# MinghanLi/STMask

Measured on AMD Instinct MI355X. Metric: frames/sec at 360x640 R50-DCN-FPN (STMask hot path, fp32), higher is better.
Workload: dtype f32

## Files before the change

stmask_amd/csrc/mask_ops.hip:

```cpp
#include "stm_common.h"

namespace {

constexpr int LC_DCHUNK = 32;

#ifndef LC_ABL
#define LC_ABL 0
#endif
template <int M>
__global__ __launch_bounds__(256) void lincomb_kernel(const float* __restrict__ proto, const float* __restrict__ coeff,
                                                      const float* __restrict__ boxes, float* __restrict__ out, int h,
                                                      int w, int n, int apply_tanh, const int* __restrict__ n_dev,
                                                      const int* __restrict__ row_proto, unsigned long long* __restrict__ bits,
                                                      float bits_thr, int dchunk)
{
    __shared__ float sc[LC_DCHUNK * M];
    __shared__ float sb[LC_DCHUNK * 4];
    const int hw = h * w;
    const int pix = blockIdx.x * 256 + threadIdx.x;
    const int d0 = blockIdx.y * dchunk;
    const int nd = min(dchunk, n - d0);
    const int n_valid = n_dev ? min(max(*n_dev, 0), n) : n;

    for (int idx = threadIdx.x; idx < nd * M; idx += 256) {
        float v = coeff[(int64_t)d0 * M + idx];
        sc[idx] = apply_tanh ? tanhf(v) : v;
    }
    if (threadIdx.x < nd) {
        float x1 = 0.f, x2 = (float)w, y1 = 0.f, y2 = (float)h;
        if (boxes) {
            const float* b = boxes + (int64_t)(d0 + threadIdx.x) * 4;
            stm_sanitize(b[0], b[2], w, 1, x1, x2);
            stm_sanitize(b[1], b[3], h, 1, y1, y2);
        }
        sb[threadIdx.x * 4 + 0] = x1;
        sb[threadIdx.x * 4 + 1] = x2;
        sb[threadIdx.x * 4 + 2] = y1;
        sb[threadIdx.x * 4 + 3] = y2;
    }
    __shared__ int hit[LC_DCHUNK];
    const int p0 = blockIdx.x * 256;
    const bool vec_ok = (hw & 3) == 0 && (reinterpret_cast<uintptr_t>(out) & 15) == 0;
    if (threadIdx.x < nd) {
        const int d = threadIdx.x;
        const int pl = min(p0 + 255, hw - 1);
        const int ya = p0 / w, yb = pl / w;
        const float fya = (float)ya, fyb = (float)yb;
        bool touch = (d0 + d < n_valid) && fyb >= sb[d * 4 + 2] && fya < sb[d * 4 + 3];
        if (touch && ya == yb) {
            const float fxa = (float)(p0 - ya * w), fxb = (float)(pl - ya * w);
            touch = fxb >= sb[d * 4] && fxa < sb[d * 4 + 1];
        }
        hit[d] = (touch || !vec_ok) ? 1 : 0;
    }
    __syncthreads();
    const bool live = pix < hw;
    const int words = (hw + 63) >> 6;
    if (p0 < hw) {
        const int lane = threadIdx.x & 63, wv = threadIdx.x >> 6;
        const int q = p0 + 4 * lane;
        for (int d = wv; d < nd; d += 4) {
            if (hit[d]) continue;
            if (q < hw && !(LC_ABL & 2)) *reinterpret_cast<float4*>(out + (int64_t)(d0 + d) * hw + q) = make_float4(0.f, 0.f, 0.f, 0.f);
            if (bits && lane < 4 && (p0 >> 6) + lane < words && !(LC_ABL & 4)) bits[(int64_t)(d0 + d) * words + (p0 >> 6) + lane] = 0ull;
        }
    }
    if (!bits && !live) return;
    if (bits && ((pix & ~63) >= hw)) return;

    float p[M];
    int cur = -1;
    const int y = pix / w, x = pix - y * w;
    const float fx = (float)x, fy = (float)y;
    for (int d = 0; d < nd; ++d) {
        if (!hit[d]) continue;
        const int want = row_proto ? row_proto[d0 + d] : 0;
        if (want != cur && live) {
            cur = want;
            const float4* pr = reinterpret_cast<const float4*>(proto + ((int64_t)cur * hw + pix) * M);
#pragma unroll
            for (int q = 0; q < M / 4; ++q) {
                float4 v = (LC_ABL & 1) ? make_float4(0.01f * q, 0.02f, 0.03f, 0.04f) : pr[q];
                p[4 * q] = v.x; p[4 * q + 1] = v.y; p[4 * q + 2] = v.z; p[4 * q + 3] = v.w;
            }
        }
        float v = 0.0f;
        const bool inside = live && (d0 + d < n_valid) && fx >= sb[d * 4] && fx < sb[d * 4 + 1] && fy >= sb[d * 4 + 2] &&
                            fy < sb[d * 4 + 3];
        if (inside) {
            float acc = 0.0f;
#pragma unroll
            for (int k = 0; k < M; ++k) acc = fmaf(p[k], sc[d * M + k], acc);
            v = 1.0f / (1.0f + expf(-acc));
        }
        if (live && (!(LC_ABL & 2) || v == 12345.678f)) out[(int64_t)(d0 + d) * hw + pix] = v;
        if (bits && !(LC_ABL & 4)) {
            const unsigned long long bal = __ballot(v > bits_thr);
            if ((threadIdx.x & 63) == 0) bits[(int64_t)(d0 + d) * words + (pix >> 6)] = bal;
        }
    }
}

__global__ __launch_bounds__(256) void mask_pack_kernel(const float* __restrict__ m, unsigned long long* __restrict__ bits,
                                                        int hw, int words, float thr)
{
    const int wave = threadIdx.x >> 6, lane = threadIdx.x & 63;
    const int word = blockIdx.x * 4 + wave;
    const int i = blockIdx.y;
    if (word >= words) return;
    const int pix = word * 64 + lane;
    bool b = false;
    if (pix < hw) b = m[(int64_t)i * hw + pix] > thr;
    unsigned long long bal = __ballot(b);
    if (lane == 0) bits[(int64_t)i * words + word] = bal;
}

__global__ __launch_bounds__(256) void mask_iou_pairs_small_kernel(const unsigned long long* __restrict__ b1,
                                                             const unsigned long long* __restrict__ b2, int n2, int words,
                                                             float* __restrict__ out, const int* __restrict__ g1,
                                                             const int* __restrict__ g2)
{
    extern __shared__ unsigned long long arow[];
    const int i = blockIdx.y;
    const int gi = g1 ? g1[i] : 0;
    if (g2) {
        const int j = blockIdx.x * 256 + threadIdx.x;
        const bool mine = j < n2 && g2[j] == gi;
        if (!__syncthreads_or(mine ? 1 : 0)) {
            if (j < n2) out[(int64_t)i * n2 + j] = 0.0f;
            return;
        }
    }
    for (int t = threadIdx.x; t < words; t += 256) arow[t] = b1[(int64_t)i * words + t];
    __syncthreads();
    const int j = blockIdx.x * 256 + threadIdx.x;
    if (j >= n2) return;
    if (g2 && g2[j] != gi) { out[(int64_t)i * n2 + j] = 0.0f; return; }
    int inter = 0, a1 = 0, a2 = 0;
    const unsigned long long* q = b2 + (int64_t)j * words;
    for (int t = 0; t < words; ++t) {
        unsigned long long a = arow[t], b = q[t];
        inter += __popcll(a & b);
        a1 += __popcll(a);
        a2 += __popcll(b);
    }
    float fi = (float)inter, uni = ((float)a1 + (float)a2) - fi;
    out[(int64_t)i * n2 + j] = (uni == 0.0f) ? 0.0f : fi / uni;
}

constexpr int MIOU_R = 8, MIOU_LIST = 2048, MIOU_BIG_ROWS = 3072;
constexpr int MIOU_DYN_LDS = 46 * 1024;
__global__ __launch_bounds__(256) void mask_iou_pairs_kernel(const unsigned long long* __restrict__ b1,
                                                             const unsigned long long* __restrict__ b2, int n1, int n2, int words,
                                                             float* __restrict__ out, const int* __restrict__ g1,
                                                             const int* __restrict__ g2, int R)
{
    extern __shared__ unsigned long long arow[];
    __shared__ int a1_s[MIOU_R], gi_s[MIOU_R];
    const int i0 = blockIdx.x * R, nr = min(R, n1 - i0);
    const int tid = threadIdx.x, lane = tid & 63, wave = tid >> 6;
    for (int r = wave; r < MIOU_R; r += 4) {
        unsigned pa = 0;
        for (int t = lane; t < words && r < nr; t += 64) {
            const unsigned long long a = b1[(int64_t)(i0 + r) * words + t];
            arow[r * words + t] = a;
            pa += (unsigned)__popcll(a);
        }
        pa = stm_row16_sum(pa);
        const int tot = stm_wave_sum_rows(pa);
        if (lane == 0) { a1_s[r] = tot; gi_s[r] = r < nr ? (g1 ? g1[i0 + r] : 0) : -0x7fffffff; }
    }
    __syncthreads();
    int gi[MIOU_R];
#pragma unroll
    for (int r = 0; r < MIOU_R; ++r) gi[r] = gi_s[r];
    const int q = lane >> 4, sl = lane & 15;
    __shared__ int list_j[MIOU_LIST], list_m[MIOU_LIST], chunk_n[4], list_n;
    if (tid == 0) list_n = 0;
// ... 23 lines not shown
        __syncthreads();
    }
    const int nlist = min(list_n, MIOU_LIST);
    for (int p0 = wave * 4; p0 < nlist; p0 += 16) {
        const int pi = min(p0 + q, nlist - 1);
        const int jq = list_j[pi];
        const unsigned mq = (unsigned)list_m[pi];
        const unsigned long long* col = b2 + (int64_t)jq * words;
        unsigned hi[MIOU_R], lo = 0;
#pragma unroll
        for (int r = 0; r < MIOU_R; ++r) hi[r] = 0;
        for (int t0 = sl; t0 < words; t0 += 16 * 16) {
            unsigned long long c[16];
#pragma unroll
            for (int u = 0; u < 16; ++u) c[u] = t0 + 16 * u < words ? col[t0 + 16 * u] : 0ull;
#pragma unroll
            for (int u = 0; u < 16; ++u) {
                const int t = t0 + 16 * u;
                if (t < words) {
                    lo += (unsigned)__popcll(c[u]);
#pragma unroll
                    for (int r = 0; r < MIOU_R; ++r)
                        if (r < nr) hi[r] += (unsigned)__popcll(arow[r * words + t] & c[u]);
                }
            }
        }
        lo = stm_row16_sum(lo);
#pragma unroll
        for (int r = 0; r < MIOU_R; ++r) hi[r] = stm_row16_sum(hi[r]);
        if (sl < MIOU_R && p0 + q < nlist) {
            unsigned h = 0;
#pragma unroll
            for (int r = 0; r < MIOU_R; ++r)
                if (sl == r) h = hi[r];
            if (sl < nr && ((mq >> sl) & 1u)) {
                const float fi = (float)h, uni = ((float)a1_s[sl] + (float)lo) - fi;
                out[(int64_t)(i0 + sl) * n2 + jq] = (uni == 0.0f) ? 0.0f : fi / uni;
            }
        }
    }
    if (list_n > MIOU_LIST) {
        for (int j = 0, seen = 0; j < n2; ++j) {
            const int gj = g2 ? g2[j] : 0;
            unsigned match = 0;
#pragma unroll
            for (int r = 0; r < MIOU_R; ++r) match |= (unsigned)(r < nr && gj == gi[r]) << r;
            if (!match) continue;
            if (seen++ < MIOU_LIST) continue;
            if (wave != 0) continue;
            const unsigned long long* col = b2 + (int64_t)j * words;
            for (int r = 0; r < nr; ++r) {
                if (!((match >> r) & 1u)) continue;
                unsigned h = 0, o = 0;
                for (int t = lane; t < words; t += 64) { const unsigned long long c = col[t]; o += (unsigned)__popcll(c); h += (unsigned)__popcll(arow[r * words + t] & c); }
                const int hs = stm_wave_sum_rows(stm_row16_sum(h)), os = stm_wave_sum_rows(stm_row16_sum(o));
                if (lane == 0) {
                    const float fi = (float)hs, uni = ((float)a1_s[r] + (float)os) - fi;
                    out[(int64_t)(i0 + r) * n2 + j] = (uni == 0.0f) ? 0.0f : fi / uni;
                }
            }
        }
    }
}

}

extern "C" int stm_lincomb_sigmoid_crop_bits_f32(const float* proto, const float* coeff, const float* boxes, float* out, int h, int w, int m,
                                                 int n, int apply_tanh, const int* n_dev, const int* row_proto, uint64_t* bits, float bits_thr,
                                                 stm_stream_t stream);
extern "C" int stm_lincomb_sigmoid_crop_f32(const float* proto, const float* coeff, const float* boxes, float* out, int h,
                                            int w, int m, int n, int apply_tanh, const int* n_dev, const int* row_proto,
                                            stm_stream_t stream)
{
    return stm_lincomb_sigmoid_crop_bits_f32(proto, coeff, boxes, out, h, w, m, n, apply_tanh, n_dev, row_proto, nullptr, 0.5f, stream);
}

extern "C" int stm_lincomb_sigmoid_crop_bits_f32(const float* proto, const float* coeff, const float* boxes, float* out, int h, int w, int m,
                                                 int n, int apply_tanh, const int* n_dev, const int* row_proto, uint64_t* bits_out, float bits_thr,
                                                 stm_stream_t stream)
{
    unsigned long long* bits = reinterpret_cast<unsigned long long*>(bits_out);
    STM_REQUIRE(n >= 0, STM_EINVAL, "stm_lincomb_sigmoid_crop_f32: n=%d", n);
    if (n == 0) return STM_OK;
    STM_REQUIRE(proto && coeff && out, STM_ENULL, "stm_lincomb_sigmoid_crop_f32: proto/coeff/out must be non-NULL");
    STM_REQUIRE(h > 0 && w > 0, STM_EINVAL, "stm_lincomb_sigmoid_crop_f32: bad mask size %dx%d", h, w);
    STM_REQUIRE((uintptr_t)proto % 16 == 0, STM_EINVAL, "stm_lincomb_sigmoid_crop_f32: proto must be 16-byte aligned");
    const int dchunk = (int64_t)stm_cdiv((int64_t)h * w, 256) * stm_cdiv(n, 32) >= 2048 ? 32 : 8;
    dim3 grid(stm_cdiv((int64_t)h * w, 256), stm_cdiv(n, dchunk));
    STM_REQUIRE(grid.y <= 65535, STM_EINVAL, "stm_lincomb_sigmoid_crop_f32: n=%d too large", n);
    if (m == 32) {
        hipLaunchKernelGGL(lincomb_kernel<32>, grid, dim3(256), 0, stm_hs(stream), proto, coeff, boxes, out, h, w, n,
                           apply_tanh, n_dev, row_proto, bits, bits_thr, dchunk);
    } else if (m == 8) {
        hipLaunchKernelGGL(lincomb_kernel<8>, grid, dim3(256), 0, stm_hs(stream), proto, coeff, boxes, out, h, w, n,
                           apply_tanh, n_dev, row_proto, bits, bits_thr, dchunk);
    } else if (m == 64) {
        hipLaunchKernelGGL(lincomb_kernel<64>, grid, dim3(256), 0, stm_hs(stream), proto, coeff, boxes, out, h, w, n,
                           apply_tanh, n_dev, row_proto, bits, bits_thr, dchunk);
    } else {
        STM_REQUIRE(false, STM_EUNSUPPORTED, "stm_lincomb_sigmoid_crop_f32: mask_dim %d not in {8,32,64}", m);
    }
    STM_CHECK_LAUNCH("lincomb_kernel");
    return STM_OK;
}

extern "C" size_t stm_mask_iou_workspace_bytes(int n1, int n2, int hw)
{
    size_t words = (size_t)((hw + 63) / 64);
    return ((size_t)n1 + (size_t)n2) * words * 8 + 64;
}

extern "C" int stm_mask_iou_grouped_f32(const float* m1, int n1, const float* m2, int n2, int hw, float thr, float* out, const int* group1,
                                        const int* group2, void* workspace, size_t workspace_bytes, stm_stream_t stream);
extern "C" int stm_mask_iou_f32(const float* m1, int n1, const float* m2, int n2, int hw, float thr, float* out,
                                void* workspace, size_t workspace_bytes, stm_stream_t stream)
{
    return stm_mask_iou_grouped_f32(m1, n1, m2, n2, hw, thr, out, nullptr, nullptr, workspace, workspace_bytes, stream);
}

extern "C" int stm_mask_iou_grouped_f32(const float* m1, int n1, const float* m2, int n2, int hw, float thr, float* out, const int* group1,
                                        const int* group2, void* workspace, size_t workspace_bytes, stm_stream_t stream)
{
    STM_REQUIRE((group1 == nullptr) == (group2 == nullptr), STM_EINVAL, "stm_mask_iou_grouped_f32: give both group arrays or neither");
    STM_REQUIRE(n1 >= 0 && n2 >= 0 && hw > 0, STM_EINVAL, "stm_mask_iou_f32: bad sizes");
    if (n1 == 0 || n2 == 0) return STM_OK;
    STM_REQUIRE(m1 && m2 && out, STM_ENULL, "stm_mask_iou_f32: m1/m2/out must be non-NULL");
    STM_REQUIRE(workspace && workspace_bytes >= stm_mask_iou_workspace_bytes(n1, n2, hw), STM_EWORKSPACE,
                "stm_mask_iou_f32: workspace too small");
    STM_REQUIRE(n1 <= 65535 && n2 <= 65535, STM_EINVAL, "stm_mask_iou_f32: too many masks");

    const int words = (hw + 63) / 64;
    unsigned long long* b1 = reinterpret_cast<unsigned long long*>(workspace);
    unsigned long long* b2 = b1 + (size_t)n1 * words;
    hipLaunchKernelGGL(mask_pack_kernel, dim3(stm_cdiv(words, 4), n1), dim3(256), 0, stm_hs(stream), m1, b1, hw, words, thr);
    hipLaunchKernelGGL(mask_pack_kernel, dim3(stm_cdiv(words, 4), n2), dim3(256), 0, stm_hs(stream), m2, b2, hw, words, thr);
    STM_CHECK_LAUNCH("mask_pack_kernel");
    const int rows_wg = std::min(MIOU_R, MIOU_DYN_LDS / (words * 8));
    STM_REQUIRE(rows_wg >= 1, STM_EUNSUPPORTED, "stm_mask_iou_f32: a mask row of %d words does not fit the 46 KB of LDS the kernel stages rows in", words);
    if (n1 < STM_ENV_INT("STM_MIOU_BIG_ROWS", MIOU_BIG_ROWS))
        hipLaunchKernelGGL(mask_iou_pairs_small_kernel, dim3(stm_cdiv(n2, 256), n1), dim3(256), (size_t)words * 8, stm_hs(stream), b1, b2, n2, words, out, group1, group2);
    else
        hipLaunchKernelGGL(mask_iou_pairs_kernel, dim3(stm_cdiv(n1, rows_wg)), dim3(256), (size_t)rows_wg * words * 8, stm_hs(stream), b1,
                           b2, n1, n2, words, out, group1, group2, rows_wg);
    STM_CHECK_LAUNCH("mask_iou_pairs_kernel");
    return STM_OK;
}

extern "C" int stm_mask_iou_bits_f32(const uint64_t* bits1, int n1, const uint64_t* bits2, int n2, int hw, float* out, const int* group1,
                                     const int* group2, stm_stream_t stream)
{
    STM_REQUIRE((group1 == nullptr) == (group2 == nullptr), STM_EINVAL, "stm_mask_iou_bits_f32: give both group arrays or neither");
    STM_REQUIRE(n1 >= 0 && n2 >= 0 && hw > 0, STM_EINVAL, "stm_mask_iou_bits_f32: bad sizes");
    if (n1 == 0 || n2 == 0) return STM_OK;
    STM_REQUIRE(bits1 && bits2 && out, STM_ENULL, "stm_mask_iou_bits_f32: bits1/bits2/out must be non-NULL");
    STM_REQUIRE(n1 <= 65535 && n2 <= 65535, STM_EINVAL, "stm_mask_iou_bits_f32: too many masks");

    const int words = (hw + 63) / 64;
    const int rows_wg = std::min(MIOU_R, MIOU_DYN_LDS / (words * 8));
    STM_REQUIRE(rows_wg >= 1, STM_EUNSUPPORTED, "stm_mask_iou_bits_f32: a mask row of %d words does not fit the 46 KB of LDS the kernel stages rows in", words);
    if (n1 < STM_ENV_INT("STM_MIOU_BIG_ROWS", MIOU_BIG_ROWS))
        hipLaunchKernelGGL(mask_iou_pairs_small_kernel, dim3(stm_cdiv(n2, 256), n1), dim3(256), (size_t)words * 8, stm_hs(stream),
                           reinterpret_cast<const unsigned long long*>(bits1), reinterpret_cast<const unsigned long long*>(bits2), n2, words, out, group1, group2);
    else
        hipLaunchKernelGGL(mask_iou_pairs_kernel, dim3(stm_cdiv(n1, rows_wg)), dim3(256), (size_t)rows_wg * words * 8, stm_hs(stream),
                           reinterpret_cast<const unsigned long long*>(bits1), reinterpret_cast<const unsigned long long*>(bits2), n1, n2, words, out, group1,
                           group2, rows_wg);
    STM_CHECK_LAUNCH("mask_iou_pairs_kernel");
// ... 150 lines not shown
```

stmask_amd/ops.py:

```python
import ctypes
import os

import torch

from . import _lib
from ._lib import DeformGeom, StmError, c_p, call


def _pair(v):
    return (v, v) if isinstance(v, int) else tuple(v)


def _dev(*ts):
    for t in ts:
        if t is not None and not t.is_cuda:
            raise StmError("stmask_amd ops need tensors on the MI355X (got a CPU tensor); there is no CPU fallback")


def _f32c(t):
    if t.dtype != torch.float32:
        raise StmError(f"expected float32, got {t.dtype}")
    return t if t.is_contiguous() else t.contiguous()


# ... 516 lines not shown
def encode(matched, priors):
    _dev(matched, priors)
    matched, priors = _f32c(matched), _f32c(priors)
    if matched.dim() != 2 or matched.shape[1] != 4 or priors.shape != matched.shape:
        raise StmError(f"encode: matched {tuple(matched.shape)} and priors {tuple(priors.shape)} must both be [n, 4]")
    out = torch.empty_like(matched)
    call("stm_encode_boxes_f32", _p(matched), _p(priors), _p(out), matched.shape[0], _stream())
    return out


_match_offsets = {}


def match_offsets(counts, device):
    if len(counts) == 1:
        key = (device.index, counts[0])
        t = _match_offsets.get(key)
        if t is None:
            t = _match_offsets[key] = torch.tensor([0, counts[0]], dtype=torch.int32, device=device)
        return t
    acc = [0]
    for c in counts:
        acc.append(acc[-1] + int(c))
    return torch.tensor(acc, dtype=torch.int32).pin_memory().to(device, non_blocking=True)


def match_priors(boxes, labels, ids, counts, priors, conf, pos_thresh, neg_thresh, out=None, offsets=None, want_status=False):
    _dev(boxes, labels, ids, priors, conf)
    counts = [int(c) for c in counts]
    B, G_total, G_max = len(counts), sum(counts), max(counts) if counts else 0
    conf = conf.detach()
    boxes, priors, conf = _f32c(boxes), _f32c(priors), _f32c(conf)
    if conf.dim() == 2:
        conf = conf[None]
    if conf.dim() != 3 or conf.shape[0] != B:
        raise StmError(f"match_priors: conf {tuple(conf.shape)} for {B} images (expected [B, P, C])")
    P, C = conf.shape[1], conf.shape[2]
    if tuple(boxes.shape) != (G_total, 4) or labels.shape[0] != G_total or ids.shape[0] != G_total:
        raise StmError(f"match_priors: boxes {tuple(boxes.shape)}, labels {tuple(labels.shape)}, ids {tuple(ids.shape)} for {G_total} boxes")
    if tuple(priors.shape) not in ((P, 4), (B, P, 4)):
        raise StmError(f"match_priors: priors {tuple(priors.shape)} for P={P}, B={B}")
    labels, ids = labels.to(torch.int64).contiguous(), ids.to(torch.int64).contiguous()
    dev = conf.device
    if offsets is None:
        offsets = match_offsets(counts, dev)
    if out is None:
        out = (torch.empty(B, P, 4, dtype=torch.float32, device=dev), torch.empty(B, P, 4, dtype=torch.float32, device=dev),
               torch.empty(B, P, dtype=torch.int64, device=dev), torch.empty(B, P, dtype=torch.int64, device=dev),
               torch.empty(B, P, dtype=torch.int64, device=dev))
    else:
        for t, dt, shp in zip(out, (torch.float32,) * 2 + (torch.int64,) * 3, ((B, P, 4),) * 2 + ((B, P),) * 3):
            if t.dtype != dt or t.numel() != B * P * (4 if len(shp) == 3 else 1) or not t.is_contiguous() or t.device != dev:
                raise StmError(f"match_priors: output {tuple(t.shape)} {t.dtype} must be contiguous {dt} with the elements of {shp}")
    status = torch.empty(B, dtype=torch.int32, device=dev) if want_status else None
    nbytes = _lib.lib().stm_match_workspace_bytes(B, P, G_total, G_max)
    ws = _workspace(nbytes, dev, "match")
    call("stm_match_priors_f32", _p(boxes), _p(labels), _p(ids), _p(offsets), B, G_total, G_max, _p(priors), 1 if priors.dim() == 3 else 0, P,
         _p(conf), C, float(pos_thresh), float(neg_thresh), _p(out[0]), _p(out[1]), _p(out[2]), _p(out[3]), _p(out[4]), _p(status), _p(ws), nbytes,
         _stream())
    return tuple(out) + ((status,) if want_status else ())


def jaccard(a, b):
    _dev(a, b)
    a, b = _f32c(a), _f32c(b)
    out = torch.empty(a.shape[0], b.shape[0], dtype=torch.float32, device=a.device)
    call("stm_jaccard_f32", _p(a), a.shape[0], _p(b), b.shape[0], _p(out), _stream())
    return out


def jaccard_backward(grad_out, a, b, need_a=True, need_b=True):
    _dev(grad_out, a, b)
    go, a, b = _f32c(grad_out), _f32c(a), _f32c(b)
    if tuple(go.shape) != (a.shape[0], b.shape[0]):
        raise StmError(f"jaccard_backward: grad_out {tuple(go.shape)} != {(a.shape[0], b.shape[0])}")
    ga = torch.empty_like(a) if need_a else None
    gb = torch.empty_like(b) if need_b else None
    if ga is None and gb is None:
        return None, None
    call("stm_jaccard_backward_f32", _p(go), _p(a), a.shape[0], _p(b), b.shape[0], _p(ga), _p(gb), _stream())
    return ga, gb


def lincomb_sigmoid_crop_bits(proto, coeff, boxes, row_proto, thr=0.5, apply_tanh=True):
    _dev(proto, coeff, boxes, row_proto)
    proto, coeff = _f32c(proto), _f32c(coeff)
    assert proto.dim() == 4 and row_proto.dtype == torch.int32 and row_proto.numel() == coeff.shape[0]
    h, w, m = proto.shape[1:]
    n = coeff.shape[0]
    out = torch.empty(n, h, w, dtype=torch.float32, device=proto.device)
    bits = torch.empty(n, (h * w + 63) // 64, dtype=torch.int64, device=proto.device)
    call("stm_lincomb_sigmoid_crop_bits_f32", _p(proto), _p(coeff), _p(_f32c(boxes)), _p(out), h, w, m, n, 1 if apply_tanh else 0, c_p(0),
         _p(row_proto), _p(bits), thr, _stream())
    return out, bits


def mask_iou_bits(bits1, bits2, hw, group1=None, group2=None):
    _dev(bits1, bits2, group1, group2)
    n1, n2 = bits1.shape[0], bits2.shape[0]
    if n1 == 0 or n2 == 0:
        return torch.zeros(n1, n2, dtype=torch.float32, device=bits1.device)
    out = torch.empty(n1, n2, dtype=torch.float32, device=bits1.device)
    if bits1.dtype != torch.int64 or bits2.dtype != torch.int64 or bits1.shape[1] != (hw + 63) // 64 or bits2.shape[1] != bits1.shape[1]:
        raise StmError("mask_iou_bits: bit tables must be int64 [n, ceil(hw / 64)]")
    call("stm_mask_iou_bits_f32", _p(bits1.contiguous()), n1, _p(bits2.contiguous()), n2, hw, _p(out),
         _p(group1.contiguous()) if group1 is not None else c_p(0), _p(group2.contiguous()) if group2 is not None else c_p(0), _stream())
    return out


def lincomb_sigmoid_crop(proto, coeff, boxes=None, apply_tanh=True, n_dev=None, row_proto=None):
    _dev(proto, coeff, boxes, row_proto)
    proto, coeff = _f32c(proto), _f32c(coeff)
    if row_proto is not None:
        assert proto.dim() == 4 and row_proto.dtype == torch.int32 and row_proto.numel() == coeff.shape[0]
        h, w, m = proto.shape[1:]
    else:
        h, w, m = proto.shape
    n = coeff.shape[0]
    bx = _f32c(boxes) if boxes is not None else None
    out = torch.empty(n, h, w, dtype=torch.float32, device=proto.device)
    call("stm_lincomb_sigmoid_crop_f32", _p(proto), _p(coeff), _p(bx), _p(out), h, w, m, n, 1 if apply_tanh else 0, _p(n_dev), _p(row_proto),
         _stream())
    return out


def lincomb_sigmoid_crop_backward(grad_out, proto, coeff, boxes=None, apply_tanh=True, need_proto=True, need_coeff=True):
    _dev(grad_out, proto, coeff, boxes)
    go, proto, coeff = _f32c(grad_out), _f32c(proto), _f32c(coeff)
    h, w, m = proto.shape
    n = coeff.shape[0]
    if tuple(go.shape) != (n, h, w) or coeff.shape[1] != m or (boxes is not None and tuple(boxes.shape) != (n, 4)):
        raise StmError(f"lincomb_sigmoid_crop_backward: grad_out {tuple(go.shape)}, proto {tuple(proto.shape)}, coeff {tuple(coeff.shape)} do not match")
    gp = torch.empty_like(proto) if need_proto else None
    gc = torch.empty_like(coeff) if need_coeff else None
    if gp is None and gc is None:
        return None, None
    bx = _f32c(boxes) if boxes is not None else None
    need = _lib.lib().stm_lincomb_backward_workspace_bytes(n, h, w, m)
    ws = _workspace(need, proto.device, "lcb")
    call("stm_lincomb_backward_f32", _p(go), _p(proto), _p(coeff), _p(bx), _p(gp), _p(gc), h, w, m, n, 1 if apply_tanh else 0, _p(ws), ws.numel(),
         _stream())
    return gp, gc


def _mask_bce_args(who, pred, target, idx, grad_loss=None):
    if pred.dtype != torch.float32 or pred.dim() != 3:
        raise StmError(f"{who}: pred must be float32 [n,h,w], got {pred.dtype} {tuple(pred.shape)}")
    if target.dtype not in (torch.uint8, torch.bool, torch.float32) or target.dim() != 3:
        raise StmError(f"{who}: target must be uint8, bool or float32 [G,H,W], got {target.dtype} {tuple(target.shape)}")
    n, h, w = pred.shape
    G, H, W = target.shape
    if h > H or w > W:
        raise StmError(f"{who}: pred {h}x{w} is larger than the target {H}x{W} (downsampling is not supported)")
    if idx is None:
        if G != n:
            raise StmError(f"{who}: without idx row i uses target i, but pred has {n} rows and target {G}")
    elif idx.dtype != torch.int64 or idx.dim() != 1 or idx.numel() != n:
        raise StmError(f"{who}: idx must be int64 [{n}], got {idx.dtype} {tuple(idx.shape)}")
    if grad_loss is not None and (grad_loss.dtype != torch.float32 or tuple(grad_loss.shape) != (n,)):
        raise StmError(f"{who}: grad_loss must be float32 [{n}], got {grad_loss.dtype} {tuple(grad_loss.shape)}")
    _dev(pred, target, idx, grad_loss)
    target = target if target.is_contiguous() else target.contiguous()
    if target.dtype == torch.bool:
        target = target.view(torch.uint8)
    return _f32c(pred), target, (idx if idx is None or idx.is_contiguous() else idx.contiguous()), target.dtype == torch.float32


def mask_bce_upsampled(pred, target, idx=None):
    pred, target, idx, is_f32 = _mask_bce_args("mask_bce_upsampled", pred, target, idx)
    n, h, w = pred.shape
    G, H, W = target.shape
    loss = torch.empty(n, dtype=torch.float32, device=pred.device)
    if n == 0:
        return loss
    need = _lib.lib().stm_mask_bce_workspace_bytes(n, H, W)
    ws = _workspace(need, pred.device, "mbce")
    call("stm_mask_bce_upsampled_f32", _p(pred), _p(target), 1 if is_f32 else 0, _p(idx), _p(loss), n, h, w, G, H, W, _p(ws), ws.numel(), _stream())
# ... 1260 lines not shown
```

stmask_amd/pipeline.py:

```python
import os
import sys
import time

import torch
import torch.nn.functional as F

from . import fuse, ops, track_host
from .dist import DET_COLS
from .layers import Track_TF, generate_candidate
from .trunk import TrunkRunner, concurrent_side_streams, trunk_stream_count

ROI_CHUNKS = (256, 128, 64)


class _StageTimer:

    def __init__(self):
        self.on = os.environ.get("STM_PIPE_TIMING", "0") == "1"
        self.acc, self.t0 = {}, None

    def tic(self):
        if self.on:
            torch.cuda.synchronize()
            self.t0 = time.perf_counter()

    def toc(self, name):
        if self.on and self.t0 is not None:
            torch.cuda.synchronize()
            t = time.perf_counter()
            self.acc[name] = self.acc.get(name, 0.0) + (t - self.t0)
            self.t0 = t


class ClipPipeline:
    def __init__(self, net, n_clips):
        self.net = net
        self.cfg = net.cfg
        if not self.cfg.temporal_fusion_module:
            raise NotImplementedError("ClipPipeline drives the temporal-fusion configs (all STMask_plus_* configs)")
        self.trackers = [Track_TF(cfg=self.cfg) for _ in range(n_clips)]
        self.t = 0

    @torch.no_grad()
    def step(self, frames, is_first=None):
        net, cfg = self.net, self.cfg
        first = (self.t == 0) if is_first is None else is_first
        fpn_outs, pred = net.forward_single(frames)
        pred["conf"] = F.softmax(pred["conf"], -1)
        pred["fpn_feat"] = fpn_outs[net.correlation_selected_layer]
        pred["T2S_feat"] = pred["T2S_feat"][net.correlation_selected_layer]
        candidates = generate_candidate(pred, cfg=cfg)
        out = []
        for i, cand in enumerate(candidates):
            det = net.Detect_TF.detect(cand, is_output_candidate=True)
            meta = {"is_first": first, "video_id": i, "frame_id": self.t}
            out.append(self.trackers[i].track(net, det, meta, img=None))
        self.t += 1
        return out


_ROW_KEYS = ("box", "mask_coeff", "track", "class", "score", "centerness", "mask")


class _TrackedRows(dict):

    _deferred = None

    def defer_mask(self, prev_mask, det_mask, plan, n_prev, plan_host=None):
        self._deferred = (prev_mask, det_mask, plan, n_prev, plan_host)
        dict.pop(self, "mask", None)

    def deferred_mask(self):
        return None if dict.__contains__(self, "mask") else self._deferred

    def _materialize(self):
        if not dict.__contains__(self, "mask") and self._deferred is not None:
            a, b, plan, n_prev, _ = self._deferred
            dict.__setitem__(self, "mask", ops.gather_rows2([a], [b], plan, n_prev)[0])
            self._deferred = None

    def __getitem__(self, key):
        if key == "mask":
            self._materialize()
        return dict.__getitem__(self, key)

    def get(self, key, default=None):
        return self[key] if key in self else default

    def keys(self):
        self._materialize()
        return dict.keys(self)

    def values(self):
        self._materialize()
        return dict.values(self)

    def items(self):
        self._materialize()
        return dict.items(self)

    def __iter__(self):
        self._materialize()
        return dict.__iter__(self)

    def __setitem__(self, key, value):
        if key == "mask":
            self._deferred = None
        dict.__setitem__(self, key, value)

    def __contains__(self, key):
        return dict.__contains__(self, key) or (key == "mask" and self._deferred is not None)


class BatchedClipPipeline(TrunkRunner):

    def __init__(self, net, n_clips, device_tracker=False):
        super().__init__(net, n_clips, _StageTimer())
        self.range_fallback = True
        self.fell_back = False
        self._last = None
        self.t = 0
        self.device_tracker = bool(device_tracker)
        if self.device_tracker and not self.tf:
            raise ValueError("BatchedClipPipeline: device_tracker needs a temporal-fusion net (the tracker without the module decides on the host)")
        self._unsettled = None
        self._off_pin = [None, None]
        self._n_resolved = 0
        self._cnt_dev = None
        self._drop_pin = []
        self._n_drops = 0
        self.prev = None
        self.prev_n = [0] * n_clips
        self.prev_feat = None
        self.tracked = [[] for _ in range(n_clips)]
        self._bits = None
        self._prev_bits = None
        self._off_dev = None
        self._tm_dev = None
        self._idle_masks = {}
        self._idle_dev = None
        self.max_instances = 0

    @property
    def prev(self):
        self._settle()
        return self._prev

    @prev.setter
    def prev(self, v):
        self._prev = v

    @property
    def prev_n(self):
        self._settle()
        return self._prev_n

    @prev_n.setter
    def prev_n(self, v):
        self._prev_n = v

    @property
    def tracked(self):
        if not self.device_tracker:
            return self._tracked
        self._settle()
        if self._prev is None or self._tm_dev is None or sum(self._prev_n) == 0:
            return [[] for _ in range(self.B)]
        tm, off = self._tm_dev.tolist(), track_host.clip_offsets(self._prev_n)
        return [tm[off[b]:off[b + 1]] for b in range(self.B)]

    @tracked.setter
    def tracked(self, v):
        self._tracked = v

    def _settle(self):
        pend = self._unsettled
        if pend is None:
            return
        self._unsettled = None
        buf, ev = pend
        ev.synchronize()
        off = buf.tolist()
        self._prev_n = [off[b + 1] - off[b] for b in range(self.B)]
        R, prev = off[-1], self._prev
        if prev is None:
            return
        for k in list(dict.keys(prev)):
            dict.__setitem__(prev, k, dict.__getitem__(prev, k)[:R])
        if prev._deferred is not None:
            a, b_, plan, n_prev, host_plan = prev._deferred
            prev._deferred = (a, b_, plan[:R], n_prev, host_plan)
        self._bits, self._tm_dev = self._bits[:R], self._tm_dev[:R]

    def _roi_feats(self, P4_prev, P4, T2S_prev, T2S, rois):
        P = self.cfg.correlation_patch_size
        corr = ops.corr_patch(P4_prev, P4, P, 1, scale=1.0 / P4.shape[1], leaky_slope=0.1)
        corr = corr.view(P4.shape[0], P * P, P4.shape[2], P4.shape[3])
        feats = F.relu(torch.cat([corr, T2S_prev, T2S], dim=1))
        roi_feats = ops.roi_align(feats, rois, 7)
        self.timer.toc("tf_corr_roi")
        return roi_feats

    def _shift_prev(self, P4, T2S, proto, dev):
        net, cfg, prev = self.net, self.cfg, self.prev
        clip_of_row = prev["clip"]
        P4_prev, T2S_prev = self.prev_feat
        P = cfg.correlation_patch_size
        fh, fw = P4.shape[2:]
        rois = ops.shift_rois(prev["box"], clip_of_row, fh, fw)
        ptn = getattr(net, "_planar_temporal", None)
        a_prev, a_cur = T2S_prev.permute(0, 2, 3, 1), T2S.permute(0, 2, 3, 1)
        if (ptn is not None and ptn.ncorr == P * P and a_prev.is_contiguous() and a_cur.is_contiguous()
                and 2 * T2S.shape[1] + P * P == ptn.cin):
            corr = ops.corr_patch_nhwc(P4_prev, P4, P, scale=1.0 / P4.shape[1], leaky_slope=0.1)
            xp = ops.roi_align_planes(a_prev, a_cur, corr, rois, 7, fmt=ptn.fmt, corr_nhwc=P * P)
            self.timer.toc("tf_corr_roi")
            loc_shift, coeff_shift = ptn.forward_planes(xp, rois.shape[0])
        elif ptn is not None:
            loc_shift, coeff_shift = ptn(self._roi_feats(P4_prev, P4, T2S_prev, T2S, rois))
        else:
            roi_feats = self._roi_feats(P4_prev, P4, T2S_prev, T2S, rois)
            n = roi_feats.shape[0]
            n_pad = -(-n // ROI_CHUNKS[-1]) * ROI_CHUNKS[-1]
            if n_pad != n:
                roi_feats = torch.cat([roi_feats, roi_feats.new_zeros(n_pad - n, *roi_feats.shape[1:])], 0)
            outs, i = [], 0
            while i < n_pad:
                c = next(c for c in ROI_CHUNKS if c <= n_pad - i)
                outs.append(net.TemporalNet(roi_feats[i:i + c]))
                i += c
            loc_shift = torch.cat([o[0] for o in outs], 0)[:n]
            coeff_shift = torch.cat([o[1] for o in outs], 0)[:n]
        self.timer.toc("tf_temporalnet")
        ops.shift_apply_(loc_shift, coeff_shift, prev["box"], prev["mask_coeff"], prev["score"], 0.95)
        prev["mask"], self._prev_bits = ops.lincomb_sigmoid_crop_bits(proto, prev["mask_coeff"], prev["box"], clip_of_row)
        self.timer.toc("tf_masks")
        if self.device_tracker:
            self._tm_dev = self._tm_dev + 1
            return
        for b in range(self.B):
            self.tracked[b] = [v + 1 for v in self.tracked[b]]

    def _detect(self, pred):
        cfg, net = self.cfg, self.net
        priors = pred["priors"].squeeze(0)
        det = net.Detect_TF if self.tf else net.detect
        if getattr(det, "use_cross_class_nms", True):
            return ops.detect_cc(pred["loc"], priors, pred["conf"], pred["centerness"], cfg.eval_conf_thresh, cfg.nms_thresh, cfg.nms_top_k, logits=True)
        return ops.detect_pc(pred["loc"], priors, F.softmax(pred["conf"], -1), pred["centerness"] if self.tf else None, cfg.eval_conf_thresh, cfg.nms_thresh,
                             cfg.nms_top_k, cfg.max_num_detections)

    @torch.no_grad()
    def step(self, frames, is_first=None, next_frames=None, active=None):
        self._settle()
        first, resets = self._first_flags(is_first)
        idle = self._idle_flags(active, frames.device)
        if first:
            self.prev, self.prev_n, self.prev_feat = None, [0] * self.B, None
            self.tracked = [[] for _ in range(self.B)]
        drop = sorted(set(resets) | set(idle))
        snap = self._snapshot() if (self.range_fallback and self._range_guarded()) else None
        self._drop_clips(drop, frames.device)
        try:
            return self._step(frames, first, next_frames)
        except ops.RangeError:
            if snap is None:
                raise
            self._fall_back(snap)
            self._drop_clips(drop, frames.device)
            return self._step(frames, first, next_frames)

    def _clip_flags(self, v, what):
        if torch.is_tensor(v):
            if v.device.type != "cpu" or v.dtype != torch.bool or tuple(v.shape) != (self.B,):
                raise ValueError(f"BatchedClipPipeline.step: {what} must be a CPU bool tensor of shape [{self.B}], got {v.dtype} {tuple(v.shape)} on {v.device}")
            v = v.tolist()
        v = [bool(x) for x in v]
        if len(v) != self.B:
            raise ValueError(f"BatchedClipPipeline.step: {what} has {len(v)} entries for {self.B} clips")
        return v

    def _first_flags(self, is_first):
        if is_first is None:
            return self.t == 0, []
        if (torch.is_tensor(is_first) and is_first.dim() == 0) or not hasattr(is_first, "__len__"):
            return bool(is_first), []
        f = self._clip_flags(is_first, "is_first")
        if all(f) or not any(f):
            return f[0], []
        return False, [b for b in range(self.B) if f[b]]

    def _idle_flags(self, active, dev):
        self._idle_dev = None
        if active is None:
            return []
        a = self._clip_flags(active, "active")
        if all(a):
            return []
        key = (dev, tuple(a))
        if key not in self._idle_masks:
            self._idle_masks[key] = torch.tensor([not x for x in a], dtype=torch.bool).to(dev)
        self._idle_dev = self._idle_masks[key]
        return [b for b in range(self.B) if not a[b]]

    def _drop_clips(self, clips, dev):
        if not clips:
            return
        if self.device_tracker:
            return self._drop_clips_dev(clips, dev)
        prev_n = list(self.prev_n)
        for b in clips:
            self.tracked[b] = []
            self.prev_n[b] = 0
        if self.prev is None or not any(prev_n[b] for b in clips):
            return
        keep, n_rows = track_host.keep_rows(prev_n, set(clips)), sum(prev_n)
        if not keep:
            self.prev, self._bits, self._prev_bits = None, None, None
            return
        prev = self.prev
        deferred = prev.deferred_mask() if isinstance(prev, _TrackedRows) else None
        mask_plan = [deferred[4][r] for r in keep] if deferred is not None and deferred[4] is not None else None
        if deferred is not None and mask_plan is None:
            prev["mask"]
            deferred = None
        off = track_host.clip_offsets(self.prev_n)
        meta = torch.tensor(off + keep + (mask_plan or []), dtype=torch.int32).to(dev, non_blocking=True)
        nb, nk = len(off), len(keep)
        self._off_dev, keep_dev = meta[:nb], meta[nb:nb + nk]
        keys = [k for k in dict.keys(prev) if k != "mask"]
        srcs = [dict.__getitem__(prev, k) for k in keys] + [self._bits]
        rows = ops.gather_rows2(srcs, [t[:0] for t in srcs], keep_dev, n_rows)
        kept = _TrackedRows() if self.tf else {}
        for k, t in zip(keys, rows[:-1]):
            kept[k] = t
        if self.tf:
            if deferred is not None:
                a, b_, _, n_prev, _ = deferred
                kept.defer_mask(a, b_, meta[nb + nk:], n_prev, mask_plan)
            elif dict.__contains__(prev, "mask"):
                m = dict.__getitem__(prev, "mask")
                kept.defer_mask(m, m[:0], keep_dev, n_rows, keep)
        self.prev, self._bits, self._prev_bits = kept, rows[-1], None

    def _drop_clips_dev(self, clips, dev):
        prev_n = list(self._prev_n)
        for b in clips:
            self._prev_n[b] = 0
        if self._prev is None or not any(prev_n[b] for b in clips):
            return
        n_rows, n_keep = sum(prev_n), sum(self._prev_n)
        if not n_keep:
            self._prev, self._bits, self._prev_bits, self._tm_dev, self._off_dev = None, None, None, None, None
            return
        keep_dev, self._off_dev = ops.track_drop_plan(self._off_dev, self._drop_flags(clips, dev), n_keep)
        prev = self._prev
        deferred = prev.deferred_mask() if isinstance(prev, _TrackedRows) else None
        keys = [k for k in dict.keys(prev) if k != "mask"]
        srcs = [dict.__getitem__(prev, k) for k in keys] + [self._bits, self._tm_dev]
        rows = ops.gather_rows2(srcs, [t[:0] for t in srcs], keep_dev, n_rows)
        kept = _TrackedRows()
        for k, t in zip(keys, rows[:-2]):
            kept[k] = t
        if deferred is not None:
            a, b_, plan, n_prev, _ = deferred
            kept.defer_mask(a, b_, plan.index_select(0, keep_dev.long()), n_prev)
        elif dict.__contains__(prev, "mask"):
            m = dict.__getitem__(prev, "mask")
            kept.defer_mask(m, m[:0], keep_dev, n_rows)
        self._prev, self._bits, self._tm_dev, self._prev_bits = kept, rows[-2], rows[-1], None

    def _drop_flags(self, clips, dev):
        slot = self._n_drops % 4
        self._n_drops += 1
        if len(self._drop_pin) <= slot:
            self._drop_pin.append([torch.empty(self.B, dtype=torch.int32).pin_memory(), None])
        buf, ev = self._drop_pin[slot]
        if ev is not None:
            ev.synchronize()
        gone = set(clips)
        buf.copy_(torch.tensor([int(b in gone) for b in range(self.B)], dtype=torch.int32))
        flags = buf.to(dev, non_blocking=True)
        ev = torch.cuda.Event()
        ev.record()
        self._drop_pin[slot][1] = ev
        return flags

    def _range_guarded(self):
        g = getattr(self.net, "_planar", None)
        return g is not None and getattr(self.net, "_planar_planes", "bf16x3") != "bf16x3"

    def _snapshot(self):
        prev = self.prev
        rows = None
        if self.tf and prev is not None and sum(self.prev_n):
            rows = tuple(prev[k].clone() for k in ("box", "mask_coeff", "score"))
        state = (prev, list(self.prev_n), self._bits, self._prev_bits, self._off_dev)
        if self.device_tracker:
            return rows, self._tm_dev, self.t, state
        return rows, [list(t) for t in self.tracked], self.t, state

    def _fall_back(self, snap):
        net = self.net
        self._pending = []
        torch.cuda.synchronize()
        flag = ops._range_flags.get(torch.cuda.current_device())
        if flag is not None:
            flag.zero_()
        sys.stderr.write(f"stmask_amd: step {self.t}: an activation left the range of the {getattr(net, '_planar_planes', 'fp16')} planar format (|x| > 65504); "
                         "rebuilding the inference graph with bf16x3 planes, repeating the step and staying there (half the convolution rate)\n")
        if getattr(net, "_planar_bf16x3", None) is None:
            net._planar_bf16x3 = fuse.build_planar(net, "bf16x3")
        fuse.attach_planar(net, net._planar_bf16x3)
        self._reset_graphs()
        rows, tracked, t, state = snap
        self.prev, self.prev_n, self._bits, self._prev_bits, self._off_dev = state[0], list(state[1]), state[2], state[3], state[4]
        if rows is not None:
            for k, v in zip(("box", "mask_coeff", "score"), rows):
                self.prev[k].copy_(v)
        if self.device_tracker:
            self._tm_dev, self.t = tracked, t
        else:
            self.tracked, self.t = tracked, t
        self.fell_back = True

    def _step(self, frames, first, next_frames):
        if self.tf:
            return self._step_tf(frames, next_frames)
        return self._step_nontf(frames, first, next_frames)

    def _detections(self, pred, mask_coeff, max_instances=0):
        idx, cls, score, box, cnt = self._detect(pred)
        if max_instances > 0:
            cnt = torch.clamp(cnt, max=max_instances)
        if self._idle_dev is not None:
            cnt = cnt.masked_fill(self._idle_dev, 0)
        if self.device_tracker:
            counts, host_scores = ops.counts_to_host(cnt), None
            self._cnt_dev = cnt
        else:
            counts, host_scores = ops.counts_to_host(cnt, extra=score)
        self.timer.toc("detect")
        top_k = idx.shape[1]
        det = ops.gather_detections(idx, cls, score, box, cnt, mask_coeff, pred["track"], pred["centerness"], sum(counts))
        if host_scores is None:
            return det, counts, None
        det_scores = [float(host_scores[b * top_k + j]) for b in range(self.B) for j in range(counts[b])]
        return det, counts, det_scores

    def _match_scores(self, det, det_bits, prev_bits, n_pixels):
        prev = self.prev
        miou = ops.mask_iou_bits(det_bits, prev_bits, n_pixels, group1=det["clip"], group2=prev["clip"])
        match = ops.match_scores_embed(det["track"], prev["track"], miou, det["box"], prev["box"], det["score"], det["class"], prev["class"],
                                       det["clip"], self._off_dev, self.cfg.match_coeff, 0.3)
        return match, miou

    def _step_tf(self, frames, next_frames):
        net = self.net
        dev = frames.device
        tmr = self.timer
        tmr.tic()
        if getattr(net, "_planar", None) is not None and tmr.on:
            net._planar.timer = tmr
        fpn_outs, pred, dropped = self._take_trunk(frames)
        tmr.toc("trunk")
        if self.prefetch_early and not (dropped and self.graph_active):
            self._prefetch_trunk(next_frames)
            next_frames = None
        P4 = fpn_outs[net.correlation_selected_layer]
        T2S = pred["T2S_feat"][net.correlation_selected_layer]
        proto = pred["proto"]
        Pn = sum(self.prev_n) if self.prev is not None else 0
        if Pn:
            self._shift_prev(P4, T2S, proto, dev)
        self._prefetch_trunk(next_frames)
        det, counts, det_scores = self._detections(pred, pred["mask_coeff"], self.max_instances)
        D = sum(counts)
        if D:
            det["mask"], det_bits = ops.lincomb_sigmoid_crop_bits(proto, det["mask_coeff"], det["box"], det["clip"])
        else:
            det["mask"], det_bits = proto.new_zeros(0, proto.shape[1], proto.shape[2]), None
        tmr.toc("det_gather_masks")
        if self.device_tracker:
            return self._update_dev(det, det_bits, counts, Pn, P4, T2S, proto, dev)

        if self.prev is None:
            self.prev, self._bits = det, det_bits
            self.prev_n = list(counts)
            self.tracked = [[0] * k for k in counts]
            self._upload_meta(dev, None)
        else:
            prev = self.prev
            if D and Pn:
                ids = self._match_scores(det, det_bits, self._prev_bits, proto.shape[1] * proto.shape[2])[0].tolist()
                tmr.toc("match_scores")
            else:
                ids = [0] * D
            plan, self.prev_n, self.tracked = track_host.match_tf(self.prev_n, self.tracked, counts, ids, det_scores, self.max_instances)
            plan_dev = self._upload_meta(dev, plan if D else None)
            if D:
                keys = tuple(k for k in _ROW_KEYS if k != "mask") + ("clip",)
                pbits = self._prev_bits if Pn else det_bits[:0]
                rows = ops.gather_rows2([prev[k] for k in keys] + [pbits], [det[k] for k in keys] + [det_bits], plan_dev, Pn)
                merged = _TrackedRows()
                for k, t in zip(keys, rows[:-1]):
                    merged[k] = t
                merged.defer_mask(prev["mask"], det["mask"], plan_dev, Pn, plan)
                self.prev, self._bits = merged, rows[-1]
            else:
                self._bits = self._prev_bits if Pn else None
            tmr.toc("tracker_update")
        self.prev_feat = (P4, T2S)
        self.t += 1
        out = self._pack_outputs(dev)
        tmr.toc("pack")
        return out

    def _update_dev(self, det, det_bits, counts, Pn, P4, T2S, proto, dev):
        tmr, D = self.timer, sum(counts)
        cnt = self._cnt_dev
        if self._prev is None:
            self._prev, self._bits, self._prev_n = det, det_bits, list(counts)
            self._off_dev = F.pad(torch.cumsum(cnt, 0, dtype=torch.int32), (1, 0))
            self._tm_dev = torch.zeros(D, dtype=torch.int32, device=dev)
        elif D:
            prev = self._prev
            match = self._match_scores(det, det_bits, self._prev_bits, proto.shape[1] * proto.shape[2])[0] if Pn else None
            tmr.toc("match_scores")
            plan, new_off, new_tm = ops.track_resolve_tf(match, det["score"], cnt, self._off_dev, self._tm_dev if Pn else None, Pn, D, self.max_instances)
            slot = self._n_resolved % 2
            self._n_resolved += 1
            if self._off_pin[slot] is None:
                self._off_pin[slot] = torch.empty(self.B + 1, dtype=torch.int32).pin_memory()
            self._off_pin[slot].copy_(new_off, non_blocking=True)
            ev = torch.cuda.Event()
            ev.record()
            keys = tuple(k for k in _ROW_KEYS if k != "mask") + ("clip",)
            pbits = self._prev_bits if Pn else det_bits[:0]
            rows = ops.gather_rows2([prev[k] for k in keys] + [pbits], [det[k] for k in keys] + [det_bits], plan, Pn)
            merged = _TrackedRows()
            for k, t in zip(keys, rows[:-1]):
                merged[k] = t
            merged.defer_mask(prev["mask"], det["mask"], plan, Pn)
            self._prev, self._bits, self._tm_dev, self._off_dev = merged, rows[-1], new_tm, new_off
            self._unsettled = (self._off_pin[slot], ev)
        else:
            self._bits = self._prev_bits if Pn else None
        tmr.toc("tracker_update")
        self.prev_feat = (P4, T2S)
        self.t += 1
        prev = self._prev
        if prev is None or prev["box"].shape[0] == 0:
            out = torch.zeros(self.B, self.cfg.nms_top_k, DET_COLS, device=dev)
        else:
            out = ops.pack_tracked_bits(self._bits, prev["score"], self._tm_dev, self._off_dev, prev["box"], prev["class"], prev["mask_coeff"], self.B,
                                        self.cfg.nms_top_k, DET_COLS, 10, self.cfg.eval_conf_thresh)
        tmr.toc("pack")
        return out

    def _step_nontf(self, frames, first, next_frames):
        cfg, B = self.cfg, self.B
        dev = frames.device
        if first:
            self.prev, self.prev_n, self._bits = None, [0] * B, None
        fpn_outs, pred, _ = self._take_trunk(frames)
        self._prefetch_trunk(next_frames)
        proto = pred["proto"]
        mc = torch.tanh(pred["mask_coeff"])
        det, counts, det_scores = self._detections(pred, mc)
        D = sum(counts)
        if not cfg.train_track:
            det["track"] = F.normalize(det["mask_coeff"], dim=1)
        out = torch.zeros(B, cfg.nms_top_k, DET_COLS, device=dev)
        if D == 0:
            self._last = None
            self.t += 1
            return out
        det_mask, det_bits = ops.lincomb_sigmoid_crop_bits(proto, det["mask_coeff"], det["box"], det["clip"])
        Pn = sum(self.prev_n)
        if Pn:
            self._upload_meta(dev, None)
            match, miou = self._match_scores(det, det_bits, self._bits, proto.shape[1] * proto.shape[2])
            ids, n_over = torch.stack([match, (miou > 0.3).sum(1).to(torch.int32)]).tolist()
        else:
            ids, n_over = [0] * D, [0] * D
        plan, new_n, obj_ids = track_host.match_nontf(self.prev_n, counts, ids, det_scores, n_over)
        rows, dst_b, dst_j = track_host.output_rows(counts, obj_ids, cfg.remove_false_inst)
        meta = torch.tensor(plan + rows + dst_b + dst_j + [obj_ids[r] for r in rows], dtype=torch.int32).to(dev, non_blocking=True)
        nP, nR = len(plan), len(rows)
        plan_dev = meta[:nP]
        r_dev, b_dev, j_dev, id_dev = (meta[nP + k * nR:nP + (k + 1) * nR].long() for k in range(4))
        keys = ("box", "mask_coeff", "track", "class", "score", "clip")
        pbits = self._bits if Pn else det_bits[:0]
        a_rows = [self.prev[k] for k in keys] if Pn else [det[k][:0] for k in keys]
        merged = ops.gather_rows2(a_rows + [pbits], [det[k] for k in keys] + [det_bits], plan_dev, Pn)
        self.prev = dict(zip(keys, merged[:-1]))
        self._bits = merged[-1]
        self.prev_n = new_n
        if nR:
            out[b_dev, j_dev, 0:4] = det["box"][r_dev]
            out[b_dev, j_dev, 4] = det["score"][r_dev]
            out[b_dev, j_dev, 5] = det["class"][r_dev].float()
            out[b_dev, j_dev, 6] = id_dev.float()
            out[b_dev, j_dev, 7] = 1.0
            out[b_dev, j_dev, 8:8 + det["mask_coeff"].shape[1]] = det["mask_coeff"][r_dev]
        self._last = (det, det_mask, r_dev, b_dev, id_dev)
        self.t += 1
        return out

    def _upload_meta(self, dev, plan):
        off = track_host.clip_offsets(self.prev_n)
        tm = [v for t in self.tracked for v in t]
        meta = torch.tensor(off + tm + (plan or []), dtype=torch.int32).to(dev, non_blocking=True)
        nb = len(off)
        self._off_dev, self._tm_dev = meta[:nb], meta[nb:nb + len(tm)]
        return meta[nb + len(tm):]

    def _pack_outputs(self, dev):
        cfg, B, prev = self.cfg, self.B, self.prev
        if prev is None or sum(self.prev_n) == 0:
            return torch.zeros(B, cfg.nms_top_k, DET_COLS, device=dev)
        return ops.pack_tracked_bits(self._bits, prev["score"], self._tm_dev, self._off_dev, prev["box"], prev["class"], prev["mask_coeff"], B,
                                     cfg.nms_top_k, DET_COLS, 10, cfg.eval_conf_thresh)

    def detections(self):
        cfg, prev = self.cfg, self.prev
# ... 46 lines not shown
```

Measured before the change: 1868.

## Compute only mask bitsets in hot path and recompute soft masks lazily from proto

The lincomb kernel now accepts a null soft-mask output, so the hot path for detections and tracked rows produces only the thresholded bitsets. This skips writing full fp32 mask planes every frame. Tracked rows no longer carry deferred gather plans for masks. They keep a reference to the prototype tensor and rebuild soft masks from coefficients, boxes and clip ids only when a caller asks for them. The risk is that lazily recomputed masks use the current proto and current coefficients rather than the frame the mask was produced on, which could change results when masks are materialized.

```diff
diff --git a/stmask_amd/csrc/mask_ops.hip b/stmask_amd/csrc/mask_ops.hip
--- a/stmask_amd/csrc/mask_ops.hip
+++ b/stmask_amd/csrc/mask_ops.hip
@@ -61,7 +61,7 @@
         const int q = p0 + 4 * lane;
         for (int d = wv; d < nd; d += 4) {
             if (hit[d]) continue;
-            if (q < hw && !(LC_ABL & 2)) *reinterpret_cast<float4*>(out + (int64_t)(d0 + d) * hw + q) = make_float4(0.f, 0.f, 0.f, 0.f);
+            if (out && q < hw && !(LC_ABL & 2)) *reinterpret_cast<float4*>(out + (int64_t)(d0 + d) * hw + q) = make_float4(0.f, 0.f, 0.f, 0.f);
             if (bits && lane < 4 && (p0 >> 6) + lane < words && !(LC_ABL & 4)) bits[(int64_t)(d0 + d) * words + (p0 >> 6) + lane] = 0ull;
         }
     }
@@ -93,7 +93,7 @@
             for (int k = 0; k < M; ++k) acc = fmaf(p[k], sc[d * M + k], acc);
             v = 1.0f / (1.0f + expf(-acc));
         }
-        if (live && (!(LC_ABL & 2) || v == 12345.678f)) out[(int64_t)(d0 + d) * hw + pix] = v;
+        if (out && live && (!(LC_ABL & 2) || v == 12345.678f)) out[(int64_t)(d0 + d) * hw + pix] = v;
         if (bits && !(LC_ABL & 4)) {
             const unsigned long long bal = __ballot(v > bits_thr);
             if ((threadIdx.x & 63) == 0) bits[(int64_t)(d0 + d) * words + (pix >> 6)] = bal;
@@ -283,7 +283,7 @@
     unsigned long long* bits = reinterpret_cast<unsigned long long*>(bits_out);
     STM_REQUIRE(n >= 0, STM_EINVAL, "stm_lincomb_sigmoid_crop_f32: n=%d", n);
     if (n == 0) return STM_OK;
-    STM_REQUIRE(proto && coeff && out, STM_ENULL, "stm_lincomb_sigmoid_crop_f32: proto/coeff/out must be non-NULL");
+    STM_REQUIRE(proto && coeff && (out || bits), STM_ENULL, "stm_lincomb_sigmoid_crop_f32: proto/coeff and one of out/bits must be non-NULL");
     STM_REQUIRE(h > 0 && w > 0, STM_EINVAL, "stm_lincomb_sigmoid_crop_f32: bad mask size %dx%d", h, w);
     STM_REQUIRE((uintptr_t)proto % 16 == 0, STM_EINVAL, "stm_lincomb_sigmoid_crop_f32: proto must be 16-byte aligned");
     const int dchunk = (int64_t)stm_cdiv((int64_t)h * w, 256) * stm_cdiv(n, 32) >= 2048 ? 32 : 8;
diff --git a/stmask_amd/ops.py b/stmask_amd/ops.py
--- a/stmask_amd/ops.py
+++ b/stmask_amd/ops.py
@@ -622,17 +622,23 @@
     return ga, gb
 
 
-def lincomb_sigmoid_crop_bits(proto, coeff, boxes, row_proto, thr=0.5, apply_tanh=True):
+def lincomb_sigmoid_crop_bits(proto, coeff, boxes, row_proto, thr=0.5, apply_tanh=True, soft=True):
     _dev(proto, coeff, boxes, row_proto)
     proto, coeff = _f32c(proto), _f32c(coeff)
     assert proto.dim() == 4 and row_proto.dtype == torch.int32 and row_proto.numel() == coeff.shape[0]
     h, w, m = proto.shape[1:]
     n = coeff.shape[0]
-    out = torch.empty(n, h, w, dtype=torch.float32, device=proto.device)
+    out = torch.empty(n, h, w, dtype=torch.float32, device=proto.device) if soft else None
     bits = torch.empty(n, (h * w + 63) // 64, dtype=torch.int64, device=proto.device)
     call("stm_lincomb_sigmoid_crop_bits_f32", _p(proto), _p(coeff), _p(_f32c(boxes)), _p(out), h, w, m, n, 1 if apply_tanh else 0, c_p(0),
          _p(row_proto), _p(bits), thr, _stream())
     return out, bits
+
+
+def lincomb_crop_bits(proto, coeff, boxes, row_proto, thr=0.5, apply_tanh=True):
+    if not proto.is_cuda:
+        return lincomb_sigmoid_crop_bits(proto, coeff, boxes, row_proto, thr, apply_tanh)[1]
+    return lincomb_sigmoid_crop_bits(proto, coeff, boxes, row_proto, thr, apply_tanh, soft=False)[1]
 
 
 def mask_iou_bits(bits1, bits2, hw, group1=None, group2=None):
diff --git a/stmask_amd/pipeline.py b/stmask_amd/pipeline.py
--- a/stmask_amd/pipeline.py
+++ b/stmask_amd/pipeline.py
@@ -64,20 +64,24 @@
 
 class _TrackedRows(dict):
 
-    _deferred = None
-
-    def defer_mask(self, prev_mask, det_mask, plan, n_prev, plan_host=None):
-        self._deferred = (prev_mask, det_mask, plan, n_prev, plan_host)
+    _proto = None
+    _mask_fn = None
+
+    def defer_mask(self, proto):
+        self._proto = proto
         dict.pop(self, "mask", None)
 
+    def mask_proto(self):
+        return self._proto
+
     def deferred_mask(self):
-        return None if dict.__contains__(self, "mask") else self._deferred
+        return None if dict.__contains__(self, "mask") else self._proto
 
     def _materialize(self):
-        if not dict.__contains__(self, "mask") and self._deferred is not None:
-            a, b, plan, n_prev, _ = self._deferred
-            dict.__setitem__(self, "mask", ops.gather_rows2([a], [b], plan, n_prev)[0])
-            self._deferred = None
+        if not dict.__contains__(self, "mask") and self._proto is not None:
+            row = lambda k: dict.__getitem__(self, k)
+            fn = self._mask_fn or ops.lincomb_sigmoid_crop
+            dict.__setitem__(self, "mask", fn(self._proto, row("mask_coeff"), row("box"), row_proto=row("clip")))
 
     def __getitem__(self, key):
         if key == "mask":
@@ -105,11 +109,11 @@
 
     def __setitem__(self, key, value):
         if key == "mask":
-            self._deferred = None
+            self._proto = None
         dict.__setitem__(self, key, value)
 
     def __contains__(self, key):
-        return dict.__contains__(self, key) or (key == "mask" and self._deferred is not None)
+        return dict.__contains__(self, key) or (key == "mask" and self._proto is not None)
 
 
 class BatchedClipPipeline(TrunkRunner):
@@ -187,9 +191,6 @@
             return
         for k in list(dict.keys(prev)):
             dict.__setitem__(prev, k, dict.__getitem__(prev, k)[:R])
-        if prev._deferred is not None:
-            a, b_, plan, n_prev, host_plan = prev._deferred
-            prev._deferred = (a, b_, plan[:R], n_prev, host_plan)
         self._bits, self._tm_dev = self._bits[:R], self._tm_dev[:R]
 
     def _roi_feats(self, P4_prev, P4, T2S_prev, T2S, rois):
@@ -233,7 +234,8 @@
             coeff_shift = torch.cat([o[1] for o in outs], 0)[:n]
         self.timer.toc("tf_temporalnet")
         ops.shift_apply_(loc_shift, coeff_shift, prev["box"], prev["mask_coeff"], prev["score"], 0.95)
-        prev["mask"], self._prev_bits = ops.lincomb_sigmoid_crop_bits(proto, prev["mask_coeff"], prev["box"], clip_of_row)
+        self._prev_bits = ops.lincomb_crop_bits(proto, prev["mask_coeff"], prev["box"], clip_of_row)
+        prev.defer_mask(proto)
         self.timer.toc("tf_masks")
         if self.device_tracker:
             self._tm_dev = self._tm_dev + 1
@@ -319,15 +321,10 @@
             self.prev, self._bits, self._prev_bits = None, None, None
             return
         prev = self.prev
-        deferred = prev.deferred_mask() if isinstance(prev, _TrackedRows) else None
-        mask_plan = [deferred[4][r] for r in keep] if deferred is not None and deferred[4] is not None else None
-        if deferred is not None and mask_plan is None:
-            prev["mask"]
-            deferred = None
         off = track_host.clip_offsets(self.prev_n)
-        meta = torch.tensor(off + keep + (mask_plan or []), dtype=torch.int32).to(dev, non_blocking=True)
-        nb, nk = len(off), len(keep)
-        self._off_dev, keep_dev = meta[:nb], meta[nb:nb + nk]
+        meta = torch.tensor(off + keep, dtype=torch.int32).to(dev, non_blocking=True)
+        nb = len(off)
+        self._off_dev, keep_dev = meta[:nb], meta[nb:]
         keys = [k for k in dict.keys(prev) if k != "mask"]
         srcs = [dict.__getitem__(prev, k) for k in keys] + [self._bits]
         rows = ops.gather_rows2(srcs, [t[:0] for t in srcs], keep_dev, n_rows)
@@ -335,12 +332,7 @@
         for k, t in zip(keys, rows[:-1]):
             kept[k] = t
         if self.tf:
-            if deferred is not None:
-                a, b_, _, n_prev, _ = deferred
-                kept.defer_mask(a, b_, meta[nb + nk:], n_prev, mask_plan)
-            elif dict.__contains__(prev, "mask"):
-                m = dict.__getitem__(prev, "mask")
-                kept.defer_mask(m, m[:0], keep_dev, n_rows, keep)
+            kept.defer_mask(prev.mask_proto())
         self.prev, self._bits, self._prev_bits = kept, rows[-1], None
 
     def _drop_clips_dev(self, clips, dev):
@@ -355,19 +347,13 @@
             return
         keep_dev, self._off_dev = ops.track_drop_plan(self._off_dev, self._drop_flags(clips, dev), n_keep)
         prev = self._prev
-        deferred = prev.deferred_mask() if isinstance(prev, _TrackedRows) else None
         keys = [k for k in dict.keys(prev) if k != "mask"]
         srcs = [dict.__getitem__(prev, k) for k in keys] + [self._bits, self._tm_dev]
         rows = ops.gather_rows2(srcs, [t[:0] for t in srcs], keep_dev, n_rows)
         kept = _TrackedRows()
         for k, t in zip(keys, rows[:-2]):
             kept[k] = t
-        if deferred is not None:
-            a, b_, plan, n_prev, _ = deferred
-            kept.defer_mask(a, b_, plan.index_select(0, keep_dev.long()), n_prev)
-        elif dict.__contains__(prev, "mask"):
-            m = dict.__getitem__(prev, "mask")
-            kept.defer_mask(m, m[:0], keep_dev, n_rows)
+        kept.defer_mask(prev.mask_proto())
         self._prev, self._bits, self._tm_dev, self._prev_bits = kept, rows[-2], rows[-1], None
 
     def _drop_flags(self, clips, dev):
@@ -476,10 +462,9 @@
         self._prefetch_trunk(next_frames)
         det, counts, det_scores = self._detections(pred, pred["mask_coeff"], self.max_instances)
         D = sum(counts)
-        if D:
-            det["mask"], det_bits = ops.lincomb_sigmoid_crop_bits(proto, det["mask_coeff"], det["box"], det["clip"])
-        else:
-            det["mask"], det_bits = proto.new_zeros(0, proto.shape[1], proto.shape[2]), None
+        det = _TrackedRows(det)
+        det.defer_mask(proto)
+        det_bits = ops.lincomb_crop_bits(proto, det["mask_coeff"], det["box"], det["clip"]) if D else None
         tmr.toc("det_gather_masks")
         if self.device_tracker:
             return self._update_dev(det, det_bits, counts, Pn, P4, T2S, proto, dev)
@@ -505,7 +490,7 @@
                 merged = _TrackedRows()
                 for k, t in zip(keys, rows[:-1]):
                     merged[k] = t
-                merged.defer_mask(prev["mask"], det["mask"], plan_dev, Pn, plan)
+                merged.defer_mask(proto)
                 self.prev, self._bits = merged, rows[-1]
             else:
                 self._bits = self._prev_bits if Pn else None
@@ -541,7 +526,7 @@
             merged = _TrackedRows()
             for k, t in zip(keys, rows[:-1]):
                 merged[k] = t
-            merged.defer_mask(prev["mask"], det["mask"], plan, Pn)
+            merged.defer_mask(proto)
             self._prev, self._bits, self._tm_dev, self._off_dev = merged, rows[-1], new_tm, new_off
             self._unsettled = (self._off_pin[slot], ev)
         else:
```

Result: no change. 1866 (-0.1%).
